# fabrii4/AutoEncoder-FFT

Hardware: AMD Instinct MI355X
Metric: frames/s fwd+bwd (FFT mode, 512x512, 4 layers) (higher is better)
Workload: dtype f32; 1 GPU; cfg3-P2: 512x512x3 frames, 4 pairs 3->8->16->32->64, 5x5, pool 2/layer, FFT mode, fwd + 1 loop-body iteration per pair (operator form); every step produces reconstructions, batch-mean gradients, updated weights and the per-pair post-update MSE partial sums -- the sums themselves are formed by the next step's gradient launch (no per-step MSE read-back inside the timed loop); frames_per_gpu=32, global_batch=32, parallelism=dp1

## Files before the change

autoencoder-fft_amd/csrc/fft_common.h:

```cpp
#pragma once
#include <hip/hip_runtime.h>
#include "internal.h"

namespace aefft {

typedef float v2f __attribute__((ext_vector_type(2)));
__device__ __forceinline__ v2f tov(float2 a) { return __builtin_bit_cast(v2f, a); }
__device__ __forceinline__ float2 tof(v2f a) { return __builtin_bit_cast(float2, a); }
__device__ __forceinline__ float2 cadd(float2 a, float2 b) { return a + b; }
__device__ __forceinline__ float2 csub(float2 a, float2 b) { return a - b; }
__device__ __forceinline__ float2 cmul(float2 a, float2 b)
{
    v2f t, r;
    const v2f av = tov(a), bv = tov(b);
    asm("v_pk_mul_f32 %0, %1, %2 op_sel:[0,0] op_sel_hi:[0,1]" : "=v"(t) : "v"(av), "v"(bv));
    asm("v_pk_fma_f32 %0, %1, %2, %3 op_sel:[1,1,0] op_sel_hi:[1,0,1] neg_lo:[0,1,0]" : "=v"(r) : "v"(av), "v"(bv), "v"(t));
    return tof(r);
}
__device__ __forceinline__ float2 cconj(float2 a) { return make_float2(a.x, -a.y); }
template <int DIR> __device__ __forceinline__ float2 mul_i(float2 a)
{
    return DIR < 0 ? make_float2(a.y, -a.x) : make_float2(-a.y, a.x);
}
template <int DIR> __device__ __forceinline__ float2 add_muli(float2 a, float2 b)
{
    v2f r;
    const v2f av = tov(a), bv = tov(b);
    if (DIR < 0) asm("v_pk_add_f32 %0, %1, %2 op_sel:[0,1] op_sel_hi:[1,0] neg_hi:[0,1]" : "=v"(r) : "v"(av), "v"(bv));
    else asm("v_pk_add_f32 %0, %1, %2 op_sel:[0,1] op_sel_hi:[1,0] neg_lo:[0,1]" : "=v"(r) : "v"(av), "v"(bv));
    return tof(r);
}
template <int DIR> __device__ __forceinline__ float2 sub_muli(float2 a, float2 b) { return add_muli<-DIR>(a, b); }

template <int R, int DIR> struct Dft;
template <int DIR> struct Dft<2, DIR> {
    static __device__ __forceinline__ void run(float2* a)
    {
        float2 t = a[0];
        a[0] = cadd(t, a[1]);
        a[1] = csub(t, a[1]);
    }
};
template <int DIR> struct Dft<4, DIR> {
    static __device__ __forceinline__ void run(float2* a)
    {
        const float2 t0 = cadd(a[0], a[2]), t1 = csub(a[0], a[2]);
        const float2 t2 = cadd(a[1], a[3]), d = csub(a[1], a[3]);
        a[0] = cadd(t0, t2); a[2] = csub(t0, t2);
        a[1] = add_muli<DIR>(t1, d); a[3] = sub_muli<DIR>(t1, d);
    }
};
template <int DIR> struct Dft<8, DIR> {
    static __device__ __forceinline__ void run(float2* a)
    {
        float2 e[4] = {a[0], a[2], a[4], a[6]};
        float2 o[4] = {a[1], a[3], a[5], a[7]};
        Dft<4, DIR>::run(e);
        Dft<4, DIR>::run(o);
        const float c = 0.70710678118654752440f;
        const float2 cc = make_float2(c, c), nc = make_float2(-c, -c);
        const float2 o1 = cc * add_muli<DIR>(o[1], o[1]);
        const float2 o3 = nc * sub_muli<DIR>(o[3], o[3]);
        a[0] = cadd(e[0], o[0]); a[4] = csub(e[0], o[0]);
        a[1] = cadd(e[1], o1);   a[5] = csub(e[1], o1);
        a[2] = add_muli<DIR>(e[2], o[2]); a[6] = sub_muli<DIR>(e[2], o[2]);
        a[3] = cadd(e[3], o3);   a[7] = csub(e[3], o3);
    }
};

__host__ __device__ constexpr int pad_idx(int n) { return n + (n >> 3); }
__host__ __device__ constexpr int pad_len(int n) { return n + (n >> 3) + 2; }

__device__ __forceinline__ unsigned px_u8(float v) { return v > 0.f ? (unsigned)fminf(roundf(v), 255.f) : 0u; }

__device__ __forceinline__ int crop_row(int i, int Nx, int Nxs)
{
    if (Nxs == Nx || i < Nxs / 2) return i;
    if (i == Nxs / 2) return Nx / 2;
    return i + Nx - Nxs;
}
__device__ __forceinline__ int padsrc_row(int r, int Nx, int Nxi)
{
    if (Nx == Nxi) return r;
    if (r < Nxi / 2) return r;
    if (r > Nx - Nxi / 2) return r - Nx + Nxi;
    if (r == Nx / 2) return Nxi / 2;
    return -1;
}

__device__ __forceinline__ float2 opin_load(const OpIn& o, long plane, int t, int Nxi, int Nyi)
{
    const int b = (int)(plane / o.D0), d = (int)(plane - (long)b * o.D0);
    const long Pc = (long)Nxi * (Nyi / 2 + 1), P0 = (long)o.Nx0 * (o.Ny0 / 2 + 1);
    const unsigned nyr = Nyi / 2 + 1, NyrB = o.Ny0 / 2 + 1;
    const unsigned i = (unsigned)t / nyr, j = (unsigned)t - i * nyr;
    const unsigned bi = i < (unsigned)Nxi / 2 ? i : (i == (unsigned)Nxi / 2 ? (unsigned)o.Nx0 / 2 : i + o.Nx0 - Nxi);
    const unsigned bj = j < nyr - 1 ? j : NyrB - 1;
    const long u = (long)bi * NyrB + bj;
    float2 acc = o.A[((long)(OPIN_COLS - 1) * o.D0 + d) * Pc + t];
    for (int jj = 0; jj < o.D0; ++jj) {
        const float2 a = o.A[((long)jj * o.D0 + d) * Pc + t], x = o.Xf[((long)b * o.D0 + jj) * P0 + u];
        acc.x += a.x * x.x - a.y * x.y; acc.y += a.x * x.y + a.y * x.x;
    }
    return acc;
}

}
```

autoencoder-fft_amd/csrc/fft_kernels.hip:

```cpp
#include "internal.h"
#include "device_util.h"
#include "fft_common.h"
#include <hip/hip_ext.h>
#include <math.h>
#include <map>
#include <mutex>
#include <vector>

namespace aefft {

__device__ float2 g_tw[TW_N];

hipError_t upload_twiddles(hipStream_t st)
{
    static std::vector<float2> host;
    if (host.empty()) {
        host.resize(TW_N);
        for (int k = 0; k < TW_N; ++k) {
            double a = -2.0 * M_PI * (double)k / (double)TW_N;
            host[k] = make_float2((float)cos(a), (float)sin(a));
        }
    }
    hipError_t e = hipMemcpyToSymbolAsync(HIP_SYMBOL(g_tw), host.data(), sizeof(float2) * TW_N, 0, hipMemcpyHostToDevice, st);
    if (e != hipSuccess) return e;
    return hipStreamSynchronize(st);
}

const float2* twiddle_table()
{
    void* p = nullptr;
    if (hipGetSymbolAddress(&p, HIP_SYMBOL(g_tw)) != hipSuccess) return nullptr;
    return static_cast<const float2*>(p);
}

bool fft_size_supported(int n) { return n >= 8 && n <= 2048 && (n & (n - 1)) == 0; }

template <int DIR> __device__ __forceinline__ float2 twid(int idx)
{
    float2 w = g_tw[idx];
    if (DIR > 0) w.y = -w.y;
    return w;
}

template <int N> __device__ __forceinline__ void pass_sync()
{
    if constexpr (N / 8 <= 64) __builtin_amdgcn_wave_barrier();
    else __syncthreads();
}

template <int N, int R, int S, int DIR>
__device__ __forceinline__ void fft_pass(float2* s, int t, float2 w1)
{
    constexpr int T = N / 8;
    constexpr int E = 8 / R;
    constexpr int n = N / S;
    float2 a[8];
#pragma unroll
    for (int v = 0; v < E; ++v) {
        const int ib = t + T * v;
#pragma unroll
        for (int tt = 0; tt < R; ++tt) a[v * R + tt] = s[pad_idx(ib + tt * (N / R))];
    }
    pass_sync<N>();
#pragma unroll
    for (int v = 0; v < E; ++v) {
        const int ib = t + T * v;
        const int p = ib / S, q = ib % S;
        Dft<R, DIR>::run(&a[v * R]);
        if constexpr (n > R) {
            static_assert(R == 8 && E == 1, "twiddled passes are radix 8");
            const float2 w2 = cmul(w1, w1), w3 = cmul(w2, w1), w4 = cmul(w2, w2);
            const float2 w5 = cmul(w4, w1), w6 = cmul(w3, w3), w7 = cmul(w4, w3);
            a[1] = cmul(a[1], w1); a[2] = cmul(a[2], w2); a[3] = cmul(a[3], w3); a[4] = cmul(a[4], w4);
            a[5] = cmul(a[5], w5); a[6] = cmul(a[6], w6); a[7] = cmul(a[7], w7);
        }
#pragma unroll
        for (int u = 0; u < R; ++u) s[pad_idx(q + S * (R * p + u))] = a[v * R + u];
    }
    if constexpr (S * R == N) __syncthreads();
    else pass_sync<N>();
}

template <int N, int DIR> struct FftTw {
    float2 w[3];
    __device__ __forceinline__ void load(int t)
    {
        constexpr int S[3] = {1, 8, 64};
#pragma unroll
        for (int i = 0; i < 3; ++i) {
            w[i] = make_float2(1.f, 0.f);
            if (N / S[i] > 8) {
                float2 v = g_tw[((t / S[i]) * S[i]) * (TW_N / N)];
                if (DIR > 0) v.y = -v.y;
                w[i] = v;
            }
        }
    }
};

template <int N, int S, int I, int DIR> struct Passes {
    static __device__ __forceinline__ void run(float2* s, int t, const FftTw<N, DIR>& tw)
    {
        constexpr int n = N / S;
        constexpr int R = n >= 8 ? 8 : n;
        fft_pass<N, R, S, DIR>(s, t, tw.w[I < 3 ? I : 2]);
        Passes<N, S * R, I + 1, DIR>::run(s, t, tw);
    }
};
template <int N, int I, int DIR> struct Passes<N, N, I, DIR> {
    static __device__ __forceinline__ void run(float2*, int, const FftTw<N, DIR>&) {}
};

template <int N, int DIR> __device__ __forceinline__ void fft_lds(float2* s, int t, const FftTw<N, DIR>& tw) { Passes<N, 1, 0, DIR>::run(s, t, tw); }

template <int N> struct RowCfg {
    static constexpr int T = N / 8;
    static constexpr int NT = T > 256 ? T : 256;
    static constexpr int G = NT / T;
    static constexpr int PL = pad_len(N);
};

template <int N, bool U8>
__global__ __launch_bounds__(RowCfg<N>::NT) void r2c_rows_kernel(const void* __restrict__ in_v, float2* __restrict__ mid,
                                                                   long npairs, int Wc)
{
    using Cfg = RowCfg<N>;
    constexpr int T = Cfg::T, NT = Cfg::NT, G = Cfg::G, PL = Cfg::PL;
    extern __shared__ float2 s[];
    const int tid = threadIdx.x;
    const int g = tid / T, t = tid % T;
    const long pair0 = (long)blockIdx.x * G;
    FftTw<N, -1> tws;
    tws.load(t);

    constexpr int NPOS = G * (N / 4) / NT;
    static_assert((G * (N / 4)) % NT == 0, "tile must be a whole number of positions per thread");
    const int live = npairs - pair0 < G ? (int)(npairs - pair0) : G;
    float4 va[NPOS], vb[NPOS];
    if constexpr (U8) {
        const unsigned* src = reinterpret_cast<const unsigned*>(static_cast<const unsigned char*>(in_v) + pair0 * 2 * N);
        unsigned wa[NPOS], wb[NPOS];
#pragma unroll
        for (int q = 0; q < NPOS; ++q) {
            const int pos = tid + q * NT;
            const int gg = pos / (N / 4), c4 = pos % (N / 4);
            const int idx = gg < live ? gg * (2 * N / 4) + c4 : c4;
            wa[q] = __builtin_nontemporal_load(&src[idx]);
            wb[q] = __builtin_nontemporal_load(&src[idx + N / 4]);
        }
#pragma unroll
        for (int q = 0; q < NPOS; ++q) {
            va[q] = make_float4((float)(wa[q] & 255u), (float)((wa[q] >> 8) & 255u), (float)((wa[q] >> 16) & 255u), (float)(wa[q] >> 24));
            vb[q] = make_float4((float)(wb[q] & 255u), (float)((wb[q] >> 8) & 255u), (float)((wb[q] >> 16) & 255u), (float)(wb[q] >> 24));
        }
    } else {
        const float4* src = reinterpret_cast<const float4*>(static_cast<const float*>(in_v) + pair0 * 2 * N);
#pragma unroll
        for (int q = 0; q < NPOS; ++q) {
            const int pos = tid + q * NT;
            const int gg = pos / (N / 4), c4 = pos % (N / 4);
            const int idx = gg < live ? gg * (2 * N / 4) + c4 : c4;
            va[q] = ld_stream(&src[idx]);
            vb[q] = ld_stream(&src[idx + N / 4]);
        }
    }
#pragma unroll
    for (int q = 0; q < NPOS; ++q) {
        const int pos = tid + q * NT;
        const int gg = pos / (N / 4), c4 = pos % (N / 4);
        if (gg < live) {
            float2* z = s + gg * PL + pad_idx(4 * c4);
            z[0] = make_float2(va[q].x, vb[q].x); z[1] = make_float2(va[q].y, vb[q].y);
            z[2] = make_float2(va[q].z, vb[q].z); z[3] = make_float2(va[q].w, vb[q].w);
        }
    }
    __syncthreads();
    fft_lds<N, -1>(s + g * PL, t, tws);

    const int half = Wc / 2, hs = 31 - __builtin_clz(half);
    float2* const obase = mid + pair0 * 2 * Wc;
    for (int it = tid; it < G * half; it += NT) {
        const int gg = it >> hs, k = (it & (half - 1)) * 2;
        if (gg >= live) continue;
        const float2* z = s + gg * PL;
        const float2 zk1 = z[pad_idx(k + 1)], zn1 = z[pad_idx(N - k - 1)];
        float2 a0, b0;
        if (k == 0) {
            const float2 z0 = z[pad_idx(0)], zh = z[pad_idx(N / 2)];
            a0 = make_float2(z0.x, zh.x); b0 = make_float2(z0.y, zh.y);
        } else {
            const float2 zk = z[pad_idx(k)], zn = z[pad_idx(N - k)];
            a0 = make_float2(0.5f * (zk.x + zn.x), 0.5f * (zk.y - zn.y)); b0 = make_float2(0.5f * (zk.y + zn.y), -0.5f * (zk.x - zn.x));
        }
        const float2 a1 = make_float2(0.5f * (zk1.x + zn1.x), 0.5f * (zk1.y - zn1.y)), b1 = make_float2(0.5f * (zk1.y + zn1.y), -0.5f * (zk1.x - zn1.x));
        float2* dst = obase + (gg * 2 * Wc + k);
        *reinterpret_cast<float4*>(dst) = make_float4(a0.x, a0.y, a1.x, a1.y);
        *reinterpret_cast<float4*>(dst + Wc) = make_float4(b0.x, b0.y, b1.x, b1.y);
    }
}

template <int N, bool SPARSE, bool U8 = false>
__global__ __launch_bounds__(RowCfg<N>::NT) void c2r_rows_kernel(const float2* __restrict__ mid, void* __restrict__ out_v,
                                                                   long npairs, int Wc, float scale)
{
    using Cfg = RowCfg<N>;
    constexpr int T = Cfg::T, NT = Cfg::NT, G = Cfg::G, PL = Cfg::PL;
    extern __shared__ float2 s[];
    const int tid = threadIdx.x;
    const int g = tid / T, t = tid % T;
    FftTw<N, +1> tws;
    tws.load(t);
    const long pair0 = (long)blockIdx.x * G;
    if constexpr (SPARSE) {
        static_assert(N >= 128, "sparse head: three radix-8 passes or more");
        const int live = npairs - pair0 < G ? (int)(npairs - pair0) : G;
        const float2* const ibase = mid + pair0 * 2 * Wc;
        const bool lo = t < Wc, hi = t > T - Wc;
        const int k = lo ? t : (hi ? T - t : 0);
        const bool ok = g < live && (lo || hi);
        const int off = ok ? g * 2 * Wc + k : 0;
        float2 A = ibase[off], B = ibase[off + Wc];
        if (!ok) { A = make_float2(0.f, 0.f); B = A; }
        const float2 zz = make_float2(0.f, 0.f);
        const float2 a0 = lo ? (t == 0 ? make_float2(A.x, B.x) : make_float2(A.x - B.y, A.y + B.x)) : zz;
        const float2 a4 = t == 0 ? make_float2(A.y, B.y) : zz;
        const float2 a7 = hi ? make_float2(A.x + B.y, -A.y + B.x) : zz;
        const float c = 0.70710678118654752440f;
        const float2 e = cadd(a0, a4), o = csub(a0, a4);
        const float2 r1 = make_float2(c * (a7.x + a7.y), c * (a7.y - a7.x));
        const float2 r2 = make_float2(a7.y, -a7.x);
        const float2 r3 = make_float2(c * (a7.y - a7.x), -c * (a7.x + a7.y));
        float2 x[8] = {cadd(e, a7), cadd(o, r1), cadd(e, r2), cadd(o, r3), csub(e, a7), csub(o, r1), csub(e, r2), csub(o, r3)};
        const float2 w1 = tws.w[0];
        const float2 w2 = cmul(w1, w1), w3 = cmul(w2, w1), w4 = cmul(w2, w2);
        const float2 w5 = cmul(w4, w1), w6 = cmul(w3, w3), w7 = cmul(w4, w3);
        x[1] = cmul(x[1], w1); x[2] = cmul(x[2], w2); x[3] = cmul(x[3], w3); x[4] = cmul(x[4], w4);
        x[5] = cmul(x[5], w5); x[6] = cmul(x[6], w6); x[7] = cmul(x[7], w7);
        float2* z = s + g * PL;
#pragma unroll
        for (int u = 0; u < 8; ++u) z[pad_idx(8 * t + u)] = x[u];
        pass_sync<N>();
        Passes<N, 8, 1, +1>::run(z, t, tws);
    } else {
    constexpr int NIT = G * (N / 4) / NT;
    static_assert((G * (N / 4)) % NT == 0, "tile must be a whole number of items per thread");
    float4 av[NIT], bv[NIT];
    const int live = npairs - pair0 < G ? (int)(npairs - pair0) : G;
    const float2* const ibase = mid + pair0 * 2 * Wc;
#pragma unroll
    for (int q = 0; q < NIT; ++q) {
        const int it = tid + q * NT;
        const int gg = it / (N / 4), k = (it % (N / 4)) * 2;
        const bool ok = gg < live && k < Wc;
        const int off = ok ? gg * 2 * Wc + k : 0;
        av[q] = ld_stream(reinterpret_cast<const float4*>(ibase + off));
        bv[q] = ld_stream(reinterpret_cast<const float4*>(ibase + off + Wc));
        if (!ok) { av[q] = make_float4(0.f, 0.f, 0.f, 0.f); bv[q] = av[q]; }
    }
#pragma unroll
    for (int q = 0; q < NIT; ++q) {
        const int it = tid + q * NT;
        const int gg = it / (N / 4), k = (it % (N / 4)) * 2;
        if (gg >= live) continue;
        float2* z = s + gg * PL;
        const float4 a = av[q], b = bv[q];
        if (k == 0) {
            z[pad_idx(0)] = make_float2(a.x, b.x);
            z[pad_idx(N / 2)] = make_float2(a.y, b.y);
        } else {
            z[pad_idx(k)] = make_float2(a.x - b.y, a.y + b.x);
            z[pad_idx(N - k)] = make_float2(a.x + b.y, -a.y + b.x);
        }
        z[pad_idx(k + 1)] = make_float2(a.z - b.w, a.w + b.z);
        z[pad_idx(N - k - 1)] = make_float2(a.z + b.w, -a.w + b.z);
    }
    __syncthreads();
    fft_lds<N, +1>(s + g * PL, t, tws);
    }

    constexpr int NQ = G * (N / 4) / NT;
    const int live = npairs - pair0 < G ? (int)(npairs - pair0) : G;
    if constexpr (U8) {
        unsigned* const orow = reinterpret_cast<unsigned*>(static_cast<unsigned char*>(out_v) + pair0 * 2 * N);
#pragma unroll
        for (int q = 0; q < NQ; ++q) {
            const int idx = tid + q * NT;
            const int gg = idx / (N / 4), n4 = idx % (N / 4);
            if (gg < live) {
                const float2* z = s + gg * PL + pad_idx(4 * n4);
                const float2 z0 = z[0], z1 = z[1], z2 = z[2], z3 = z[3];
                const unsigned wa = px_u8(z0.x * scale) | px_u8(z1.x * scale) << 8 | px_u8(z2.x * scale) << 16 | px_u8(z3.x * scale) << 24;
                const unsigned wb = px_u8(z0.y * scale) | px_u8(z1.y * scale) << 8 | px_u8(z2.y * scale) << 16 | px_u8(z3.y * scale) << 24;
                __builtin_nontemporal_store(wa, &orow[(gg * 2) * (N / 4) + n4]);
                __builtin_nontemporal_store(wb, &orow[(gg * 2 + 1) * (N / 4) + n4]);
            }
        }
        return;
    }
    float* const orow = static_cast<float*>(out_v) + pair0 * 2 * N;
#pragma unroll
    for (int q = 0; q < NQ; ++q) {
        const int idx = tid + q * NT;
        const int gg = idx / (N / 4), n = (idx % (N / 4)) * 4;
        if (gg < live) {
            const float2* z = s + gg * PL + pad_idx(n);
            const float2 z0 = z[0], z1 = z[1], z2 = z[2], z3 = z[3];
            st_stream(reinterpret_cast<float4*>(orow + (gg * 2) * N + n), make_float4(z0.x * scale, z1.x * scale, z2.x * scale, z3.x * scale));
            st_stream(reinterpret_cast<float4*>(orow + (gg * 2 + 1) * N + n), make_float4(z0.y * scale, z1.y * scale, z2.y * scale, z3.y * scale));
        }
    }
}

template <int N, int CW>
__global__ __launch_bounds__(CW* N / 8) void fwd_cols_kernel(const float2* __restrict__ mid, float2* __restrict__ out,
                                                              int Wc, int Nxs)
{
    constexpr int T = N / 8, NT = CW * T, PL = pad_len(N);
    extern __shared__ float2 s[];
    const int tid = threadIdx.x;
    FftTw<N, -1> tws;
    tws.load(tid % T);
    const long plane = blockIdx.x;
    const int c0 = blockIdx.y * CW;

    const float2* src = mid + plane * N * (long)Wc + c0;
    constexpr int NLD = N * (CW / 2) / NT;
    float4 val[NLD];
#pragma unroll
    for (int k = 0; k < NLD; ++k) {
        const int it = tid + k * NT;
        const float4* ptr = reinterpret_cast<const float4*>(src + ((it / (CW / 2)) * Wc + 2 * (it % (CW / 2))));
        if constexpr (CW * sizeof(float2) >= 128) val[k] = ld_stream(ptr);
        else val[k] = *ptr;
    }
#pragma unroll
    for (int k = 0; k < NLD; ++k) {
        const int it = tid + k * NT;
        const int r = it / (CW / 2), c2 = it % (CW / 2);
        s[(2 * c2) * PL + pad_idx(r)] = make_float2(val[k].x, val[k].y);
        s[(2 * c2 + 1) * PL + pad_idx(r)] = make_float2(val[k].z, val[k].w);
    }
    __syncthreads();
    fft_lds<N, -1>(s + (tid / T) * PL, tid % T, tws);

    const int Nyrs = Wc + 1;
    float2* dst = out + plane * Nxs * (long)Nyrs;
    for (int it = tid; it < Nxs * CW; it += NT) {
        const int i = it / CW, c = it % CW;
        const int si = crop_row(i, N, Nxs);
        const float2 z = s[c * PL + pad_idx(si)];
        const int col = c0 + c;
        if (col == 0) {
            const float2 zn = s[pad_idx((N - si) % N)];
            dst[i * Nyrs] = make_float2(0.5f * (z.x + zn.x), 0.5f * (z.y - zn.y));
            dst[i * Nyrs + Wc] = make_float2(0.5f * (z.y + zn.y), -0.5f * (z.x - zn.x));
        } else {
            dst[i * Nyrs + col] = z;
        }
    }
}

template <int N, int CW>
__global__ __launch_bounds__(CW* N / 8) void inv_cols_kernel(const float2* __restrict__ in, float2* __restrict__ mid,
                                                              int Wc, int Nxi, const OpIn op)
{
    constexpr int T = N / 8, NT = CW * T, PL = pad_len(N);
    extern __shared__ float2 s[];
    const int tid = threadIdx.x;
    FftTw<N, +1> tws;
    tws.load(tid % T);
    const long plane = blockIdx.x;
    const int c0 = blockIdx.y * CW;
    const int Nyri = Wc + 1;
    const float2* src = in + plane * Nxi * (long)Nyri;
    auto ld = [&](long t) { return op.A ? opin_load(op, plane, (int)t, Nxi, 2 * Wc) : src[t]; };

    float2* dcs = s + CW * PL;
    float2* nys = dcs + Nxi;
    if (Nxi < N) {
        for (int it = tid; it < CW * PL; it += NT) s[it] = make_float2(0.f, 0.f);
        __syncthreads();
    }
    constexpr int NLD = 8;
    float2 v[NLD], w[NLD];
    const int nsrc = Nxi * CW;
#pragma unroll
    for (int k = 0; k < NLD; ++k) {
        if (k * NT < nsrc) {
            const int it = min(tid + k * NT, nsrc - 1);
            const int sr = it / CW, c = it % CW;
            v[k] = ld((long)sr * Nyri + c0 + c);
            w[k] = (c0 + c == 0) ? ld((long)sr * Nyri + Wc) : make_float2(0.f, 0.f);
        }
    }
#pragma unroll
    for (int k = 0; k < NLD; ++k) {
        const int it = tid + k * NT;
        if (it < nsrc) {
            const int sr = it / CW, c = it % CW;
            if (c0 + c == 0) { dcs[sr] = v[k]; nys[sr] = w[k]; }
            else {
                const int r = Nxi == N ? sr : (sr < Nxi / 2 ? sr : (sr == Nxi / 2 ? N / 2 : sr + N - Nxi));
                s[c * PL + pad_idx(r)] = v[k];
            }
        }
    }
    if (c0 == 0) {
        __syncthreads();
        for (int r = tid; r < N; r += NT) {
            const int sr = padsrc_row(r, N, Nxi), sm = padsrc_row((N - r) % N, N, Nxi);
            const float2 zz = make_float2(0.f, 0.f);
            const float2 d0 = sr >= 0 ? dcs[sr] : zz, n0 = sr >= 0 ? nys[sr] : zz, d1 = sm >= 0 ? dcs[sm] : zz, n1 = sm >= 0 ? nys[sm] : zz;
            const float2 dc = make_float2(0.5f * (d0.x + d1.x), 0.5f * (d0.y - d1.y));
            const float2 ny = make_float2(0.5f * (n0.x + n1.x), 0.5f * (n0.y - n1.y));
            s[pad_idx(r)] = make_float2(dc.x - ny.y, dc.y + ny.x);
        }
    }
    __syncthreads();
    fft_lds<N, +1>(s + (tid / T) * PL, tid % T, tws);

    float2* dst = mid + plane * N * (long)Wc + c0;
    for (int it = tid; it < N * (CW / 2); it += NT) {
        const int r = it / (CW / 2), c2 = it % (CW / 2);
        const float2 a = s[(2 * c2) * PL + pad_idx(r)], b = s[(2 * c2 + 1) * PL + pad_idx(r)];
        *reinterpret_cast<float4*>(dst + (long)r * Wc + 2 * c2) = make_float4(a.x, a.y, b.x, b.y);
    }
}

template <int M> struct BluCfg {
    static constexpr int T = M / 8;
    static constexpr int NT = T > 256 ? T : 256;
    static constexpr int G = NT / T;
    static constexpr int PL = pad_len(M);
};

template <int M, int MODE>
__global__ __launch_bounds__(BluCfg<M>::NT) void bluestein_rows_kernel(const void* __restrict__ in_, void* __restrict__ out_, const float2* __restrict__ tab,
                                                                        long nrows, int n, float scale)
{
    using Cfg = BluCfg<M>;
    constexpr int T = Cfg::T, NT = Cfg::NT, G = Cfg::G, PL = Cfg::PL;
    extern __shared__ float2 s[];
    const int tid = threadIdx.x, g = tid / T, t = tid % T;
    const long row = (long)blockIdx.x * G + g;
    const bool live = row < nrows;
    FftTw<M, -1> twf;
    FftTw<M, +1> twi;
    twf.load(t); twi.load(t);
    float2* z = s + g * PL;
    const float2* const bhat = tab;
    const float2* const w = tab + M;
    const int nh = n / 2 + 1;
    for (int j = t; j < M; j += T) {
        float2 v = make_float2(0.f, 0.f);
        if (live && j < n) {
            if (MODE == 0) v = reinterpret_cast<const float2*>(in_)[row * n + j];
            else if (MODE == 1) v = make_float2(reinterpret_cast<const float*>(in_)[row * n + j], 0.f);
            else {
                const float2* X = reinterpret_cast<const float2*>(in_) + row * nh;
                if (j < nh) { v = X[j]; if (j == 0 || 2 * j == n) v.y = 0.f; }
                else { v = X[n - j]; v.y = -v.y; }
            }
            v = cmul(v, w[j]);
        }
        z[pad_idx(j)] = v;
    }
    __syncthreads();
    fft_lds<M, -1>(z, t, twf);
    for (int j = t; j < M; j += T) z[pad_idx(j)] = cmul(z[pad_idx(j)], bhat[j]);
    __syncthreads();
    fft_lds<M, +1>(z, t, twi);
    if (!live) return;
    const float sc = scale / (float)M;
    const int nout = MODE == 1 ? nh : n;
    for (int k = t; k < nout; k += T) {
        float2 v = cmul(z[pad_idx(k)], w[k]);
        if (MODE == 2) reinterpret_cast<float*>(out_)[row * n + k] = v.x * sc;
        else reinterpret_cast<float2*>(out_)[row * nout + k] = make_float2(v.x * sc, v.y * sc);
    }
}

__global__ __launch_bounds__(256) void transpose_c_kernel(const float2* __restrict__ in, float2* __restrict__ out, int R, int C)
{
    __shared__ float2 tile[32][33];
    const long plane = blockIdx.z;
    const int r0 = blockIdx.y * 32, c0 = blockIdx.x * 32;
    const int tx = threadIdx.x % 32, ty = threadIdx.x / 32;
    for (int k = ty; k < 32; k += 8) if (r0 + k < R && c0 + tx < C) tile[k][tx] = in[(plane * R + r0 + k) * C + c0 + tx];
    __syncthreads();
    for (int k = ty; k < 32; k += 8) if (c0 + k < C && r0 + tx < R) out[(plane * C + c0 + k) * R + r0 + tx] = tile[tx][k];
}

size_t fft_mid_elems(long planes, int Nx, int Wc) { return (size_t)planes * Nx * Wc; }

template <typename K> static hipError_t allow_lds(K kernel, size_t bytes)
{
    if (bytes <= 64 * 1024) return hipSuccess;
    return hipFuncSetAttribute(reinterpret_cast<const void*>(kernel), hipFuncAttributeMaxDynamicSharedMemorySize, (int)bytes);
}

template <int N> static hipError_t run_r2c_rows(const void* in, float2* mid, long npairs, int Wc, hipStream_t st, bool in_u8)
{
    using Cfg = RowCfg<N>;
    const size_t lds = sizeof(float2) * (Cfg::G * Cfg::PL);
    hipError_t e = in_u8 ? allow_lds(r2c_rows_kernel<N, true>, lds) : allow_lds(r2c_rows_kernel<N, false>, lds);
    if (e != hipSuccess) return e;
    const long blocks = (npairs + Cfg::G - 1) / Cfg::G;
    if (in_u8) r2c_rows_kernel<N, true><<<dim3((unsigned)blocks), dim3(Cfg::NT), lds, st>>>(in, mid, npairs, Wc);
    else r2c_rows_kernel<N, false><<<dim3((unsigned)blocks), dim3(Cfg::NT), lds, st>>>(in, mid, npairs, Wc);
    return hipGetLastError();
}
template <int N, bool SPARSE, bool U8> static hipError_t run_c2r_rows_as(const float2* mid, void* out, long npairs, int Wc, float scale, hipStream_t st)
{
    using Cfg = RowCfg<N>;
    const size_t lds = sizeof(float2) * (Cfg::G * Cfg::PL);
    const long blocks = (npairs + Cfg::G - 1) / Cfg::G;
    hipError_t e = allow_lds(c2r_rows_kernel<N, SPARSE, U8>, lds);
    if (e != hipSuccess) return e;
    c2r_rows_kernel<N, SPARSE, U8><<<dim3((unsigned)blocks), dim3(Cfg::NT), lds, st>>>(mid, out, npairs, Wc, scale);
    return hipGetLastError();
}
template <int N> static hipError_t run_c2r_rows(const float2* mid, void* out, long npairs, int Wc, float scale, hipStream_t st, bool out_u8)
{
    if constexpr (N >= 128) {
        if (Wc <= N / 16)
            return out_u8 ? run_c2r_rows_as<N, true, true>(mid, out, npairs, Wc, scale, st) : run_c2r_rows_as<N, true, false>(mid, out, npairs, Wc, scale, st);
    }
    return out_u8 ? run_c2r_rows_as<N, false, true>(mid, out, npairs, Wc, scale, st) : run_c2r_rows_as<N, false, false>(mid, out, npairs, Wc, scale, st);
}
template <int N, int CW> static hipError_t run_fwd_cols(const float2* mid, float2* out, long planes, int Wc, int Nxs, hipStream_t st, hipEvent_t done)
{
    const size_t lds = sizeof(float2) * (CW * pad_len(N));
    hipError_t e = allow_lds(fwd_cols_kernel<N, CW>, lds);
    if (e != hipSuccess) return e;
    if (done) hipExtLaunchKernelGGL((fwd_cols_kernel<N, CW>), dim3((unsigned)planes, Wc / CW), dim3(CW * N / 8), lds, st, nullptr, done, 0, mid, out, Wc, Nxs);
    else fwd_cols_kernel<N, CW><<<dim3((unsigned)planes, Wc / CW), dim3(CW * N / 8), lds, st>>>(mid, out, Wc, Nxs);
    return hipGetLastError();
}
static OpIn g_opin_none{};
template <int N, int CW> static hipError_t run_inv_cols(const float2* in, float2* mid, long planes, int Wc, int Nxi, hipStream_t st, const OpIn& op = g_opin_none)
{
    const size_t lds = sizeof(float2) * (CW * pad_len(N) + 2 * Nxi);
    hipError_t e = allow_lds(inv_cols_kernel<N, CW>, lds);
    if (e != hipSuccess) return e;
    inv_cols_kernel<N, CW><<<dim3((unsigned)planes, Wc / CW), dim3(CW * N / 8), lds, st>>>(in, mid, Wc, Nxi, op);
    return hipGetLastError();
}

template <int N, bool FWD> static hipError_t cols_dispatch(const float2* a, float2* b, long planes, int Wc, int Nother, hipStream_t st, const OpIn& op = g_opin_none, hipEvent_t done = nullptr)
{
    constexpr int CWMAX = (8192 / N) < 16 ? (8192 / N) : 16;
    int cw = CWMAX;
    while (cw > Wc) cw >>= 1;
    if (!FWD) while (cw > 4 && planes * (Wc / cw) < 256) cw >>= 1;
#define AEFFT_CW_CASE(C)                                                                                   \
    if constexpr (C <= CWMAX) {                                                                             \
        if (cw == C) return FWD ? run_fwd_cols<N, C>(a, b, planes, Wc, Nother, st, done) : run_inv_cols<N, C>(a, b, planes, Wc, Nother, st, op); \
    }
    AEFFT_CW_CASE(16) AEFFT_CW_CASE(8) AEFFT_CW_CASE(4)
#undef AEFFT_CW_CASE
    return hipErrorInvalidValue;
}

#define AEFFT_N_SWITCH(n, CALL)                       \
    switch (n) {                                      \
    case 8: { constexpr int NN = 8; CALL; }           \
    case 16: { constexpr int NN = 16; CALL; }         \
    case 32: { constexpr int NN = 32; CALL; }         \
    case 64: { constexpr int NN = 64; CALL; }         \
    case 128: { constexpr int NN = 128; CALL; }       \
    case 256: { constexpr int NN = 256; CALL; }       \
    case 512: { constexpr int NN = 512; CALL; }       \
    case 1024: { constexpr int NN = 1024; CALL; }     \
    case 2048: { constexpr int NN = 2048; CALL; }     \
    default: e = hipErrorInvalidValue;                \
    }

bool fft_size_supported_any(int n) { return fft_size_supported(n) || (n >= 8 && n <= 1024 && (n & 1) == 0); }
static int blu_m(int n) { int m = 16; while (m < 2 * n - 1) m *= 2; return m; }
struct BluKey { int dev, n, dir; bool operator<(const BluKey& o) const { return dev != o.dev ? dev < o.dev : (n != o.n ? n < o.n : dir < o.dir); } };
#define AEFFT_M_SWITCH(m, CALL)                      \
    switch (m) {                                      \
    case 16: { constexpr int MM = 16; CALL; }         \
    case 32: { constexpr int MM = 32; CALL; }         \
    case 64: { constexpr int MM = 64; CALL; }         \
    case 128: { constexpr int MM = 128; CALL; }       \
    case 256: { constexpr int MM = 256; CALL; }       \
    case 512: { constexpr int MM = 512; CALL; }       \
    case 1024: { constexpr int MM = 1024; CALL; }     \
    case 2048: { constexpr int MM = 2048; CALL; }     \
    default: e = hipErrorInvalidValue;                \
    }
static std::mutex g_blu_mu;
static std::vector<float2> blu_host_table(int n, int dir)
{
    const int M = blu_m(n);
    std::vector<double> wr(n), wi(n), cr(M), ci(M);
    for (int j = 0; j < n; ++j) {
        const long q = ((long)j * j) % (2L * n);
        wr[j] = cos(M_PI * (double)q / n); wi[j] = dir * sin(M_PI * (double)q / n);
    }
    for (int m = 0; m < M; ++m) { cr[m] = cos(2.0 * M_PI * m / M); ci[m] = -sin(2.0 * M_PI * m / M); }
    std::vector<float2> t(M + n);
    for (int k = 0; k < M; ++k) {
        double ar = 0.0, ai = 0.0;
        for (int j = 0; j < M; ++j) {
            const int jj = j < n ? j : (M - j < n ? M - j : -1);
            if (jj < 0) continue;
            const double br = wr[jj], bi = -wi[jj];
            const int m = (int)(((long)j * k) % M);
            ar += br * cr[m] - bi * ci[m]; ai += br * ci[m] + bi * cr[m];
        }
        t[k] = make_float2((float)ar, (float)ai);
    }
    for (int j = 0; j < n; ++j) t[M + j] = make_float2((float)wr[j], (float)wi[j]);
    return t;
}
static hipError_t blu_table(int n, int dir, const float2** out)
{
    static std::map<BluKey, float2*> cache;
    int dev = 0;
    hipError_t e = hipGetDevice(&dev);
    if (e != hipSuccess) return e;
    const BluKey key{dev, n, dir};
    std::lock_guard<std::mutex> lock(g_blu_mu);
    auto it = cache.find(key);
    if (it == cache.end()) {
        const std::vector<float2> host = blu_host_table(n, dir);
        float2* p = nullptr;
        e = hipMalloc(&p, sizeof(float2) * host.size());
        if (e != hipSuccess) return e;
        e = hipMemcpy(p, host.data(), sizeof(float2) * host.size(), hipMemcpyHostToDevice);
        if (e != hipSuccess) { (void)hipFree(p); return e; }
        it = cache.emplace(key, p).first;
    }
    *out = it->second;
    return hipSuccess;
}
template <int M, int MODE> static hipError_t run_blu_rows(const void* in, void* out, const float2* tab, long nrows, int n, float scale, hipStream_t st)
{
    using Cfg = BluCfg<M>;
    const size_t lds = sizeof(float2) * (size_t)Cfg::G * Cfg::PL;
    hipError_t e = allow_lds(bluestein_rows_kernel<M, MODE>, lds);
    if (e != hipSuccess) return e;
    const long blocks = (nrows + Cfg::G - 1) / Cfg::G;
    if (blocks >= (1L << 31)) return hipErrorInvalidValue;
    bluestein_rows_kernel<M, MODE><<<dim3((unsigned)blocks), dim3(Cfg::NT), lds, st>>>(in, out, tab, nrows, n, scale);
    return hipGetLastError();
}
static hipError_t blu_rows(int mode, const void* in, void* out, long nrows, int n, int dir, float scale, hipStream_t st)
{
    const float2* tab = nullptr;
    hipError_t e = blu_table(n, dir, &tab);
    if (e != hipSuccess) return e;
    const int M = blu_m(n);
    if (mode == 0) { AEFFT_M_SWITCH(M, e = (run_blu_rows<MM, 0>(in, out, tab, nrows, n, scale, st)); break) }
    else if (mode == 1) { AEFFT_M_SWITCH(M, e = (run_blu_rows<MM, 1>(in, out, tab, nrows, n, scale, st)); break) }
    else { AEFFT_M_SWITCH(M, e = (run_blu_rows<MM, 2>(in, out, tab, nrows, n, scale, st)); break) }
    return e;
}
static hipError_t transpose_c(const float2* in, float2* out, long planes, int R, int C, hipStream_t st)
{
    constexpr long ZMAX = 65535;
    for (long p0 = 0; p0 < planes; p0 += ZMAX) {
        const long np = planes - p0 < ZMAX ? planes - p0 : ZMAX;
        const long off = p0 * R * (long)C;
        transpose_c_kernel<<<dim3((C + 31) / 32, (R + 31) / 32, (unsigned)np), 256, 0, st>>>(in + off, out + off, R, C);
        hipError_t e = hipGetLastError();
        if (e != hipSuccess) return e;
    }
    return hipSuccess;
}
size_t fft_any_ws_elems(long planes, int Nx, int Ny) { return (size_t)planes * Nx * (Ny / 2 + 1); }
hipError_t launch_r2c_any(const float* in, float2* out, float2* w1, float2* w2, long planes, int Nx, int Ny, hipStream_t st)
{
    if (!fft_size_supported_any(Nx) || !fft_size_supported_any(Ny) || Nx > 1024 || Ny > 1024) return hipErrorInvalidValue;
    if (planes <= 0) return hipSuccess;
    const int Nyr = Ny / 2 + 1;
    hipError_t e = blu_rows(1, in, w1, planes * Nx, Ny, -1, 1.f, st);
    if (e == hipSuccess) e = transpose_c(w1, w2, planes, Nx, Nyr, st);
    if (e == hipSuccess) e = blu_rows(0, w2, w1, planes * Nyr, Nx, -1, 1.f, st);
    if (e == hipSuccess) e = transpose_c(w1, out, planes, Nyr, Nx, st);
    return e;
}
hipError_t launch_c2r_any(const float2* in, float* out, float2* w1, float2* w2, long planes, int Nx, int Ny, float scale, hipStream_t st)
{
    if (!fft_size_supported_any(Nx) || !fft_size_supported_any(Ny) || Nx > 1024 || Ny > 1024) return hipErrorInvalidValue;
    if (planes <= 0) return hipSuccess;
    const int Nyr = Ny / 2 + 1;
    hipError_t e = transpose_c(in, w1, planes, Nx, Nyr, st);
    if (e == hipSuccess) e = blu_rows(0, w1, w2, planes * Nyr, Nx, +1, 1.f, st);
    if (e == hipSuccess) e = transpose_c(w2, w1, planes, Nyr, Nx, st);
    if (e == hipSuccess) e = blu_rows(2, w1, out, planes * Nx, Ny, +1, scale, st);
    return e;
}

static bool rows_pow2(int Ny, int Wc) { return fft_size_supported(Ny) && Wc >= 4 && (Wc & (Wc - 1)) == 0; }
static bool cols_pow2(int Nx, int Wc) { return fft_size_supported(Nx) && Wc >= 4 && ((Wc & (Wc - 1)) == 0 || Wc % 16 == 0); }
static bool axis_ok(int n) { return fft_size_supported(n) || fft_size_mixed(n); }

hipError_t launch_r2c(const void* in, float2* out, float2* mid, long planes, int Nx, int Ny, int Nxs, int Nys, hipStream_t st, hipEvent_t done, bool in_u8)
{
    if (!fft_size_supported(Nx) || !fft_size_supported(Ny) || Nxs > Nx || Nys > Ny || Nys < 8 || Nxs < 2 || (Nys & (Nys - 1)) || (Nxs & 1)) {
        if (!axis_ok(Nx) || !axis_ok(Ny) || Nxs > Nx || Nys > Ny || Nxs < 2 || Nys < 2 || (Nxs & 1) || (Nys & 1)) return hipErrorInvalidValue;
        if (planes <= 0) return hipSuccess;
        const int Wc = Nys / 2;
        const long npairs = planes * Nx / 2;
        hipError_t e = hipSuccess;
        if (in) {
            if (rows_pow2(Ny, Wc)) { AEFFT_N_SWITCH(Ny, e = run_r2c_rows<NN>(in, mid, npairs, Wc, st, in_u8); break) }
            else e = launch_mix_r2c_rows(in, mid, npairs, Ny, Wc, st, in_u8);
            if (e != hipSuccess) return e;
        }
        if (out) {
            if (cols_pow2(Nx, Wc)) { AEFFT_N_SWITCH(Nx, e = (cols_dispatch<NN, true>(mid, out, planes, Wc, Nxs, st, g_opin_none, done)); break) }
            else e = launch_mix_fwd_cols(mid, out, planes, Nx, Wc, Nxs, st, done);
        }
        return e;
    }
    if (planes <= 0) return hipSuccess;
    const int Wc = Nys / 2;
    const long npairs = planes * Nx / 2;
    hipError_t e = hipSuccess;
    if (in) {
        AEFFT_N_SWITCH(Ny, e = run_r2c_rows<NN>(in, mid, npairs, Wc, st, in_u8); break)
        if (e != hipSuccess) return e;
    }
    if (out) {
        AEFFT_N_SWITCH(Nx, e = (cols_dispatch<NN, true>(mid, out, planes, Wc, Nxs, st, g_opin_none, done)); break)
    }
    return e;
}

hipError_t launch_c2r(const float2* in, void* out, float2* mid, long planes, int Nxi, int Nyi, int Nx, int Ny, float scale, hipStream_t st, const OpIn* opin,
                      bool out_u8)
{
    const OpIn op = opin ? *opin : g_opin_none;
    if ((Nxi == Nx) != (Nyi == Ny)) return hipErrorInvalidValue;
    if (!fft_size_supported(Nx) || !fft_size_supported(Ny) || Nxi > Nx || Nyi > Ny || Nyi < 8 || Nxi < 2 || (Nyi & 1) || (Nxi & 1)) {
        if (!axis_ok(Nx) || !axis_ok(Ny) || Nxi > Nx || Nyi > Ny || Nxi < 2 || Nyi < 2 || (Nxi & 1) || (Nyi & 1)) return hipErrorInvalidValue;
        if (planes <= 0) return hipSuccess;
        const int Wc = Nyi / 2;
        const long npairs = planes * Nx / 2;
        hipError_t e = hipSuccess;
        if (in || op.A) {
            if (cols_pow2(Nx, Wc)) { AEFFT_N_SWITCH(Nx, e = (cols_dispatch<NN, false>(in, mid, planes, Wc, Nxi, st, op)); break) }
            else e = launch_mix_inv_cols(in, mid, planes, Nx, Wc, Nxi, st, op.A ? &op : nullptr);
            if (e != hipSuccess) return e;
        }
        if (out) {
            if (rows_pow2(Ny, Wc)) { AEFFT_N_SWITCH(Ny, e = run_c2r_rows<NN>(mid, out, npairs, Wc, scale, st, out_u8); break) }
            else e = launch_mix_c2r_rows(mid, out, npairs, Ny, Wc, scale, st, out_u8);
        }
        return e;
    }
    if (planes <= 0) return hipSuccess;
    const int Wc = Nyi / 2;
    const long npairs = planes * Nx / 2;
    hipError_t e = hipSuccess;
    if (in || op.A) {
        AEFFT_N_SWITCH(Nx, e = (cols_dispatch<NN, false>(in, mid, planes, Wc, Nxi, st, op)); break)
        if (e != hipSuccess) return e;
    }
    if (out) {
        AEFFT_N_SWITCH(Ny, e = run_c2r_rows<NN>(mid, out, npairs, Wc, scale, st, out_u8); break)
    }
    return e;
}

}
```

Measured before the change: 220,900 frames/s.

## Prune FFT passes for cropped outputs and sparse inputs in row/column kernels

Adds a banded final radix-8 pass that computes and stores only the output bins kept after cropping (N=64/512) in the forward row and column FFTs. It also adds a sparse-input path for the inverse column FFT, used when only a few input rows are nonzero, so the first radix-8 pass runs from three live inputs. The existing sparse first-pass code is factored into a shared helper. This cuts arithmetic and LDS stores in those FFT stages, at the cost of more template instantiations and dispatch branches.

```diff
diff --git a/autoencoder-fft_amd/csrc/fft_common.h b/autoencoder-fft_amd/csrc/fft_common.h
--- a/autoencoder-fft_amd/csrc/fft_common.h
+++ b/autoencoder-fft_amd/csrc/fft_common.h
@@ -68,6 +68,24 @@
     }
 };
 
+template <int DIR> struct Dft8Band {
+    static __device__ __forceinline__ void run(float2* a)
+    {
+        float2 e[4] = {a[0], a[2], a[4], a[6]};
+        float2 o[4] = {a[1], a[3], a[5], a[7]};
+        Dft<4, DIR>::run(e);
+        Dft<4, DIR>::run(o);
+        const float c = 0.70710678118654752440f;
+        const float2 cc = make_float2(c, c), nc = make_float2(-c, -c);
+        const float2 o1 = cc * add_muli<DIR>(o[1], o[1]);
+        const float2 o3 = nc * sub_muli<DIR>(o[3], o[3]);
+        a[0] = cadd(e[0], o[0]); a[4] = csub(e[0], o[0]);
+        a[1] = cadd(e[1], o1);
+        a[6] = sub_muli<DIR>(e[2], o[2]);
+        a[7] = csub(e[3], o3);
+    }
+};
+
 __host__ __device__ constexpr int pad_idx(int n) { return n + (n >> 3); }
 __host__ __device__ constexpr int pad_len(int n) { return n + (n >> 3) + 2; }
 
diff --git a/autoencoder-fft_amd/csrc/fft_kernels.hip b/autoencoder-fft_amd/csrc/fft_kernels.hip
--- a/autoencoder-fft_amd/csrc/fft_kernels.hip
+++ b/autoencoder-fft_amd/csrc/fft_kernels.hip
@@ -48,7 +48,7 @@
     else __syncthreads();
 }
 
-template <int N, int R, int S, int DIR>
+template <int N, int R, int S, int DIR, bool CROP = false>
 __device__ __forceinline__ void fft_pass(float2* s, int t, float2 w1)
 {
     constexpr int T = N / 8;
@@ -62,6 +62,14 @@
         for (int tt = 0; tt < R; ++tt) a[v * R + tt] = s[pad_idx(ib + tt * (N / R))];
     }
     pass_sync<N>();
+    if constexpr (CROP && S * R == N) {
+        static_assert(R == 8 && S == T, "the banded last pass is radix 8 (N = 64, 512): p = 0, q = t, no twiddles");
+        Dft8Band<DIR>::run(a);
+        s[pad_idx(t)] = a[0]; s[pad_idx(t + S)] = a[1]; s[pad_idx(t + 6 * S)] = a[6]; s[pad_idx(t + 7 * S)] = a[7];
+        if (t == 0) s[pad_idx(4 * S)] = a[4];
+        __syncthreads();
+        return;
+    }
 #pragma unroll
     for (int v = 0; v < E; ++v) {
         const int ib = t + T * v;
@@ -98,20 +106,38 @@
     }
 };
 
-template <int N, int S, int I, int DIR> struct Passes {
+template <int N, int S, int I, int DIR, bool CROP = false> struct Passes {
     static __device__ __forceinline__ void run(float2* s, int t, const FftTw<N, DIR>& tw)
     {
         constexpr int n = N / S;
         constexpr int R = n >= 8 ? 8 : n;
-        fft_pass<N, R, S, DIR>(s, t, tw.w[I < 3 ? I : 2]);
-        Passes<N, S * R, I + 1, DIR>::run(s, t, tw);
+        fft_pass<N, R, S, DIR, CROP>(s, t, tw.w[I < 3 ? I : 2]);
+        Passes<N, S * R, I + 1, DIR, CROP>::run(s, t, tw);
     }
 };
-template <int N, int I, int DIR> struct Passes<N, N, I, DIR> {
+template <int N, int I, int DIR, bool CROP> struct Passes<N, N, I, DIR, CROP> {
     static __device__ __forceinline__ void run(float2*, int, const FftTw<N, DIR>&) {}
 };
-
-template <int N, int DIR> __device__ __forceinline__ void fft_lds(float2* s, int t, const FftTw<N, DIR>& tw) { Passes<N, 1, 0, DIR>::run(s, t, tw); }
+constexpr bool last_pass_radix8(int n) { return n == 64 || n == 512; }
+
+template <int N, int DIR, bool CROP = false> __device__ __forceinline__ void fft_lds(float2* s, int t, const FftTw<N, DIR>& tw) { Passes<N, 1, 0, DIR, CROP>::run(s, t, tw); }
+
+template <int N> __device__ __forceinline__ void sparse_first_pass(float2* z, int t, float2 a0, float2 a4, float2 a7, float2 w1)
+{
+    const float c = 0.70710678118654752440f;
+    const float2 e = cadd(a0, a4), o = csub(a0, a4);
+    const float2 r1 = make_float2(c * (a7.x + a7.y), c * (a7.y - a7.x));
+    const float2 r2 = make_float2(a7.y, -a7.x);
+    const float2 r3 = make_float2(c * (a7.y - a7.x), -c * (a7.x + a7.y));
+    float2 x[8] = {cadd(e, a7), cadd(o, r1), cadd(e, r2), cadd(o, r3), csub(e, a7), csub(o, r1), csub(e, r2), csub(o, r3)};
+    const float2 w2 = cmul(w1, w1), w3 = cmul(w2, w1), w4 = cmul(w2, w2);
+    const float2 w5 = cmul(w4, w1), w6 = cmul(w3, w3), w7 = cmul(w4, w3);
+    x[1] = cmul(x[1], w1); x[2] = cmul(x[2], w2); x[3] = cmul(x[3], w3); x[4] = cmul(x[4], w4);
+    x[5] = cmul(x[5], w5); x[6] = cmul(x[6], w6); x[7] = cmul(x[7], w7);
+#pragma unroll
+    for (int u = 0; u < 8; ++u) z[pad_idx(8 * t + u)] = x[u];
+    pass_sync<N>();
+}
 
 template <int N> struct RowCfg {
     static constexpr int T = N / 8;
@@ -120,7 +146,7 @@
     static constexpr int PL = pad_len(N);
 };
 
-template <int N, bool U8>
+template <int N, bool U8, bool CROP = false>
 __global__ __launch_bounds__(RowCfg<N>::NT) void r2c_rows_kernel(const void* __restrict__ in_v, float2* __restrict__ mid,
                                                                    long npairs, int Wc)
 {
@@ -175,7 +201,7 @@
         }
     }
     __syncthreads();
-    fft_lds<N, -1>(s + g * PL, t, tws);
+    fft_lds<N, -1, CROP>(s + g * PL, t, tws);
 
     const int half = Wc / 2, hs = 31 - __builtin_clz(half);
     float2* const obase = mid + pair0 * 2 * Wc;
@@ -225,21 +251,8 @@
         const float2 a0 = lo ? (t == 0 ? make_float2(A.x, B.x) : make_float2(A.x - B.y, A.y + B.x)) : zz;
         const float2 a4 = t == 0 ? make_float2(A.y, B.y) : zz;
         const float2 a7 = hi ? make_float2(A.x + B.y, -A.y + B.x) : zz;
-        const float c = 0.70710678118654752440f;
-        const float2 e = cadd(a0, a4), o = csub(a0, a4);
-        const float2 r1 = make_float2(c * (a7.x + a7.y), c * (a7.y - a7.x));
-        const float2 r2 = make_float2(a7.y, -a7.x);
-        const float2 r3 = make_float2(c * (a7.y - a7.x), -c * (a7.x + a7.y));
-        float2 x[8] = {cadd(e, a7), cadd(o, r1), cadd(e, r2), cadd(o, r3), csub(e, a7), csub(o, r1), csub(e, r2), csub(o, r3)};
-        const float2 w1 = tws.w[0];
-        const float2 w2 = cmul(w1, w1), w3 = cmul(w2, w1), w4 = cmul(w2, w2);
-        const float2 w5 = cmul(w4, w1), w6 = cmul(w3, w3), w7 = cmul(w4, w3);
-        x[1] = cmul(x[1], w1); x[2] = cmul(x[2], w2); x[3] = cmul(x[3], w3); x[4] = cmul(x[4], w4);
-        x[5] = cmul(x[5], w5); x[6] = cmul(x[6], w6); x[7] = cmul(x[7], w7);
         float2* z = s + g * PL;
-#pragma unroll
-        for (int u = 0; u < 8; ++u) z[pad_idx(8 * t + u)] = x[u];
-        pass_sync<N>();
+        sparse_first_pass<N>(z, t, a0, a4, a7, tws.w[0]);
         Passes<N, 8, 1, +1>::run(z, t, tws);
     } else {
     constexpr int NIT = G * (N / 4) / NT;
@@ -311,7 +324,7 @@
     }
 }
 
-template <int N, int CW>
+template <int N, int CW, bool CROP = false>
 __global__ __launch_bounds__(CW* N / 8) void fwd_cols_kernel(const float2* __restrict__ mid, float2* __restrict__ out,
                                                               int Wc, int Nxs)
 {
@@ -341,7 +354,7 @@
         s[(2 * c2 + 1) * PL + pad_idx(r)] = make_float2(val[k].z, val[k].w);
     }
     __syncthreads();
-    fft_lds<N, -1>(s + (tid / T) * PL, tid % T, tws);
+    fft_lds<N, -1, CROP>(s + (tid / T) * PL, tid % T, tws);
 
     const int Nyrs = Wc + 1;
     float2* dst = out + plane * Nxs * (long)Nyrs;
@@ -360,7 +373,7 @@
     }
 }
 
-template <int N, int CW>
+template <int N, int CW, bool SPARSE = false>
 __global__ __launch_bounds__(CW* N / 8) void inv_cols_kernel(const float2* __restrict__ in, float2* __restrict__ mid,
                                                               int Wc, int Nxi, const OpIn op)
 {
@@ -375,6 +388,43 @@
     const float2* src = in + plane * Nxi * (long)Nyri;
     auto ld = [&](long t) { return op.A ? opin_load(op, plane, (int)t, Nxi, 2 * Wc) : src[t]; };
 
+    if constexpr (SPARSE) {
+    static_assert(N >= 128, "sparse head: Nxi <= N/16 rows, and a compact grid has 8 rows or more");
+    const int c = tid / T, t = tid % T, col = c0 + c, h = Nxi / 2;
+    const bool lo = t < h, hi = t > T - h;
+    const int sr = lo ? t : t - T + Nxi;
+    float2* z = s + c * PL;
+    float2* park = s + CW * PL;
+    int idx, slot;
+    if (col != 0) {
+        idx = ((lo || hi) ? sr : (t == T / 2 ? h : 0)) * Nyri + col;
+        slot = t == T / 2 ? c * PL + pad_idx(0) : -1;
+    } else {
+        idx = t < Nxi ? t * Nyri : (t < 2 * Nxi ? (t - Nxi) * Nyri + Wc : 0);
+        slot = t < 2 * Nxi ? CW * PL + t : -1;
+    }
+    const float2 v = ld(idx);
+    if (slot >= 0) s[slot] = v;
+    pass_sync<N>();
+    const float2 zz = make_float2(0.f, 0.f);
+    float2 x = v, a4 = zz;
+    if (col != 0) {
+        if (t == 0) a4 = z[pad_idx(0)];
+    } else {
+        auto sym = [&](int r) {
+            const int rm = (Nxi - r) % Nxi;
+            const float2 d0 = park[r], d1 = park[rm], n0 = park[Nxi + r], n1 = park[Nxi + rm];
+            const float2 dc = make_float2(0.5f * (d0.x + d1.x), 0.5f * (d0.y - d1.y));
+            const float2 ny = make_float2(0.5f * (n0.x + n1.x), 0.5f * (n0.y - n1.y));
+            return make_float2(dc.x - ny.y, dc.y + ny.x);
+        };
+        if (lo || hi) x = sym(sr);
+        if (t == 0) a4 = sym(h);
+    }
+    const float2 a0 = lo ? x : zz, a7 = hi ? x : zz;
+    sparse_first_pass<N>(z, t, a0, a4, a7, tws.w[0]);
+    Passes<N, 8, 1, +1>::run(z, t, tws);
+    } else {
     float2* dcs = s + CW * PL;
     float2* nys = dcs + Nxi;
     if (Nxi < N) {
@@ -418,6 +468,7 @@
     }
     __syncthreads();
     fft_lds<N, +1>(s + (tid / T) * PL, tid % T, tws);
+    }
 
     float2* dst = mid + plane * N * (long)Wc + c0;
     for (int it = tid; it < N * (CW / 2); it += NT) {
@@ -499,16 +550,23 @@
     return hipFuncSetAttribute(reinterpret_cast<const void*>(kernel), hipFuncAttributeMaxDynamicSharedMemorySize, (int)bytes);
 }
 
-template <int N> static hipError_t run_r2c_rows(const void* in, float2* mid, long npairs, int Wc, hipStream_t st, bool in_u8)
+template <int N, bool U8, bool CROP> static hipError_t run_r2c_rows_as(const void* in, float2* mid, long npairs, int Wc, hipStream_t st)
 {
     using Cfg = RowCfg<N>;
     const size_t lds = sizeof(float2) * (Cfg::G * Cfg::PL);
-    hipError_t e = in_u8 ? allow_lds(r2c_rows_kernel<N, true>, lds) : allow_lds(r2c_rows_kernel<N, false>, lds);
+    hipError_t e = allow_lds(r2c_rows_kernel<N, U8, CROP>, lds);
     if (e != hipSuccess) return e;
     const long blocks = (npairs + Cfg::G - 1) / Cfg::G;
-    if (in_u8) r2c_rows_kernel<N, true><<<dim3((unsigned)blocks), dim3(Cfg::NT), lds, st>>>(in, mid, npairs, Wc);
-    else r2c_rows_kernel<N, false><<<dim3((unsigned)blocks), dim3(Cfg::NT), lds, st>>>(in, mid, npairs, Wc);
+    r2c_rows_kernel<N, U8, CROP><<<dim3((unsigned)blocks), dim3(Cfg::NT), lds, st>>>(in, mid, npairs, Wc);
     return hipGetLastError();
+}
+template <int N> static hipError_t run_r2c_rows(const void* in, float2* mid, long npairs, int Wc, hipStream_t st, bool in_u8)
+{
+    if constexpr (last_pass_radix8(N)) {
+        if (Wc <= N / 4)
+            return in_u8 ? run_r2c_rows_as<N, true, true>(in, mid, npairs, Wc, st) : run_r2c_rows_as<N, false, true>(in, mid, npairs, Wc, st);
+    }
+    return in_u8 ? run_r2c_rows_as<N, true, false>(in, mid, npairs, Wc, st) : run_r2c_rows_as<N, false, false>(in, mid, npairs, Wc, st);
 }
 template <int N, bool SPARSE, bool U8> static hipError_t run_c2r_rows_as(const float2* mid, void* out, long npairs, int Wc, float scale, hipStream_t st)
 {
@@ -528,23 +586,37 @@
     }
     return out_u8 ? run_c2r_rows_as<N, false, true>(mid, out, npairs, Wc, scale, st) : run_c2r_rows_as<N, false, false>(mid, out, npairs, Wc, scale, st);
 }
+template <int N, int CW, bool CROP> static hipError_t run_fwd_cols_as(const float2* mid, float2* out, long planes, int Wc, int Nxs, hipStream_t st, hipEvent_t done)
+{
+    const size_t lds = sizeof(float2) * (CW * pad_len(N));
+    hipError_t e = allow_lds(fwd_cols_kernel<N, CW, CROP>, lds);
+    if (e != hipSuccess) return e;
+    if (done) hipExtLaunchKernelGGL((fwd_cols_kernel<N, CW, CROP>), dim3((unsigned)planes, Wc / CW), dim3(CW * N / 8), lds, st, nullptr, done, 0, mid, out, Wc, Nxs);
+    else fwd_cols_kernel<N, CW, CROP><<<dim3((unsigned)planes, Wc / CW), dim3(CW * N / 8), lds, st>>>(mid, out, Wc, Nxs);
+    return hipGetLastError();
+}
 template <int N, int CW> static hipError_t run_fwd_cols(const float2* mid, float2* out, long planes, int Wc, int Nxs, hipStream_t st, hipEvent_t done)
 {
-    const size_t lds = sizeof(float2) * (CW * pad_len(N));
-    hipError_t e = allow_lds(fwd_cols_kernel<N, CW>, lds);
+    if constexpr (last_pass_radix8(N)) {
+        if (Nxs <= N / 2) return run_fwd_cols_as<N, CW, true>(mid, out, planes, Wc, Nxs, st, done);
+    }
+    return run_fwd_cols_as<N, CW, false>(mid, out, planes, Wc, Nxs, st, done);
+}
+static OpIn g_opin_none{};
+template <int N, int CW, bool SPARSE> static hipError_t run_inv_cols_as(const float2* in, float2* mid, long planes, int Wc, int Nxi, hipStream_t st, const OpIn& op)
+{
+    const size_t lds = sizeof(float2) * (CW * pad_len(N) + 2 * Nxi);
+    hipError_t e = allow_lds(inv_cols_kernel<N, CW, SPARSE>, lds);
     if (e != hipSuccess) return e;
-    if (done) hipExtLaunchKernelGGL((fwd_cols_kernel<N, CW>), dim3((unsigned)planes, Wc / CW), dim3(CW * N / 8), lds, st, nullptr, done, 0, mid, out, Wc, Nxs);
-    else fwd_cols_kernel<N, CW><<<dim3((unsigned)planes, Wc / CW), dim3(CW * N / 8), lds, st>>>(mid, out, Wc, Nxs);
+    inv_cols_kernel<N, CW, SPARSE><<<dim3((unsigned)planes, Wc / CW), dim3(CW * N / 8), lds, st>>>(in, mid, Wc, Nxi, op);
     return hipGetLastError();
 }
-static OpIn g_opin_none{};
 template <int N, int CW> static hipError_t run_inv_cols(const float2* in, float2* mid, long planes, int Wc, int Nxi, hipStream_t st, const OpIn& op = g_opin_none)
 {
-    const size_t lds = sizeof(float2) * (CW * pad_len(N) + 2 * Nxi);
-    hipError_t e = allow_lds(inv_cols_kernel<N, CW>, lds);
-    if (e != hipSuccess) return e;
-    inv_cols_kernel<N, CW><<<dim3((unsigned)planes, Wc / CW), dim3(CW * N / 8), lds, st>>>(in, mid, Wc, Nxi, op);
-    return hipGetLastError();
+    if constexpr (N >= 128) {
+        if (Nxi <= N / 16) return run_inv_cols_as<N, CW, true>(in, mid, planes, Wc, Nxi, st, op);
+    }
+    return run_inv_cols_as<N, CW, false>(in, mid, planes, Wc, Nxi, st, op);
 }
 
 template <int N, bool FWD> static hipError_t cols_dispatch(const float2* a, float2* b, long planes, int Wc, int Nother, hipStream_t st, const OpIn& op = g_opin_none, hipEvent_t done = nullptr)
```

After: 218,900 frames/s. About the same (-0.9%).
